# jscant/PointVS

Measured on AMD Instinct MI355X. Metric: protein-ligand graphs/sec fwd+bwd (+Adam step), 3-layer EGNN ch=32, ~2k nodes r=10A, higher is better.
Workload: dtype f32

## Files before the change

### pointvs_amd/csrc/graph_prepare.hip

```cpp
#include "common.h"
#include "profile.h"
#include <hipcub/hipcub.hpp>

namespace {

__global__ void k_extract(const int64_t* __restrict__ ei, const int64_t* __restrict__ ea, int A,
                          int N, int E, int32_t* row32, int32_t* col32, int32_t* ids,
                          uint8_t* etype_in, int32_t* status) {
    int e = blockIdx.x * blockDim.x + threadIdx.x;
    if (e >= E) return;
    int64_t r = ei[e], c = ei[(size_t)E + e];
    int bad = 0;
    if (r < 0 || r >= N || c < 0 || c >= N) { bad |= 1; r = 0; c = 0; }
    row32[e] = (int32_t)r;
    col32[e] = (int32_t)c;
    ids[e] = e;
    if (A > 0) {
        int hot = -1, ones = 0, other = 0;
        for (int a = 0; a < A; ++a) {
            int64_t v = ea[(size_t)e * A + a];
            if (v == 1) { ones++; hot = a; }
            else if (v != 0) other = 1;
        }
        if (ones != 1 || other) { bad |= 2; if (hot < 0) hot = 0; }
        etype_in[e] = (uint8_t)hot;
    }
    if (bad) atomicOr(status, bad);
}

__global__ void k_gather_sorted(const int32_t* __restrict__ perm, const int32_t* __restrict__ col32,
                                const uint8_t* __restrict__ etype_in, int E, int32_t* col,
                                uint8_t* etype, int32_t* iota) {
    int p = blockIdx.x * blockDim.x + threadIdx.x;
    if (p >= E) return;
    int e = perm[p];
    col[p] = col32[e];
    if (etype) etype[p] = etype_in[e];
    iota[p] = p;
}

__global__ void k_lower_bounds(const int32_t* __restrict__ keys, int E, int N, int32_t* ptr,
                               float* inv_deg) {
    int r = blockIdx.x * blockDim.x + threadIdx.x;
    if (r > N) return;
    auto lb = [&](int key) {
        int lo = 0, hi = E;
        while (lo < hi) {
            int mid = (lo + hi) >> 1;
            if (keys[mid] < key) lo = mid + 1; else hi = mid;
        }
        return lo;
    };
    int p0 = lb(r);
    ptr[r] = p0;
    if (inv_deg && r < N) {
        int deg = lb(r + 1) - p0;
        inv_deg[r] = 1.0f / (float)(deg > 1 ? deg : 1);
    }
}

int key_bits(int n) {
    int b = 1;
    while ((1ll << b) < (long long)n) ++b;
    return b;
}

size_t sort_temp_bytes(int E, int bits) {
    size_t bytes = 0;
    hipcub::DeviceRadixSort::SortPairs(nullptr, bytes, (const int32_t*)nullptr, (int32_t*)nullptr,
                                       (const int32_t*)nullptr, (int32_t*)nullptr, E, 0, bits, 0);
    return bytes;
}

struct PrepWs {
    int32_t *row32, *col32, *ids, *iota, *keys_tmp;
    uint8_t* etype_in;
    void* sort_tmp;
    size_t sort_bytes;
};

size_t carve(PvsArena& a, int N, int E, PrepWs* w) {
    size_t e = (size_t)(E > 0 ? E : 1);
    PrepWs t;
    t.row32 = a.take<int32_t>(e);
    t.col32 = a.take<int32_t>(e);
    t.ids = a.take<int32_t>(e);
    t.iota = a.take<int32_t>(e);
    t.keys_tmp = a.take<int32_t>(e);
    t.etype_in = a.take<uint8_t>(e);
    t.sort_bytes = sort_temp_bytes(E > 0 ? E : 1, key_bits(N > 1 ? N : 2));
    t.sort_tmp = a.take<char>(t.sort_bytes);
    if (w) *w = t;
    return a.off;
}

}

extern "C" size_t pvs_graph_prepare_workspace_bytes(int32_t n_nodes, int32_t n_edges) {
    PvsArena a(nullptr, 0);
    return carve(a, n_nodes, n_edges, nullptr) + 256;
}

extern "C" int pvs_graph_prepare(const int64_t* edge_index, const int64_t* edge_attr,
                                 int32_t n_edge_attr, int32_t N, int32_t E, int32_t* rowptr,
                                 int32_t* row, int32_t* col, uint8_t* etype, int32_t* perm,
                                 int32_t* colptr, int32_t* cedge, float* inv_deg, int32_t* status,
                                 void* workspace, size_t workspace_bytes, pvs_stream_t stream_) {
    hipStream_t stream = (hipStream_t)stream_;
    PVS_REQUIRE(N > 0 && E >= 0, "pvs_graph_prepare: bad sizes N=%d E=%d", N, E);
    PVS_REQUIRE(n_edge_attr >= 0 && n_edge_attr <= 255, "pvs_graph_prepare: bad n_edge_attr %d",
                n_edge_attr);
    PVS_REQUIRE(n_edge_attr == 0 || E == 0 || (edge_attr && etype), "pvs_graph_prepare: edge_attr/etype NULL");
    PVS_REQUIRE((colptr == nullptr) == (cedge == nullptr), "pvs_graph_prepare: colptr and cedge go together");
    PvsArena arena(workspace, workspace_bytes);
    PrepWs w;
    carve(arena, N, E, &w);
    PVS_REQUIRE(arena.ok(), "pvs_graph_prepare: workspace too small (%zu < %zu)", workspace_bytes,
                arena.off);
    PvsProfScope prof(stream, PVS_PROF_PREPARE);
    PVS_CHECK_HIP(hipMemsetAsync(status, 0, sizeof(int32_t), stream));
    const int bits = key_bits(N > 1 ? N : 2);
    const int T = 256;
    if (E > 0) {
        k_extract<<<(E + T - 1) / T, T, 0, stream>>>(edge_index, edge_attr, n_edge_attr, N, E,
                                                     w.row32, w.col32, w.ids, w.etype_in, status);
        PVS_CHECK_LAUNCH();
        size_t tb = w.sort_bytes;
        PVS_CHECK_HIP(hipcub::DeviceRadixSort::SortPairs(w.sort_tmp, tb, w.row32, row, w.ids, perm,
                                                         E, 0, bits, stream));
        k_gather_sorted<<<(E + T - 1) / T, T, 0, stream>>>(perm, w.col32, w.etype_in, E, col,
                                                           n_edge_attr ? etype : nullptr, w.iota);
        PVS_CHECK_LAUNCH();
        if (cedge) {
            tb = w.sort_bytes;
            PVS_CHECK_HIP(hipcub::DeviceRadixSort::SortPairs(w.sort_tmp, tb, col, w.keys_tmp, w.iota,
                                                             cedge, E, 0, bits, stream));
        }
    }
    k_lower_bounds<<<(N + 1 + T - 1) / T, T, 0, stream>>>(row, E, N, rowptr, inv_deg);
    PVS_CHECK_LAUNCH();
    if (cedge) {
        k_lower_bounds<<<(N + 1 + T - 1) / T, T, 0, stream>>>(w.keys_tmp, E, N, colptr, nullptr);
        PVS_CHECK_LAUNCH();
    }
    return 0;
}

namespace {

__device__ __forceinline__ int graph_of_edge(const int32_t* __restrict__ edge_ptr, int n_graphs, int e, int E,
                                             int edges_per_thread = 1) {
    __shared__ int g_first;
    if (threadIdx.x == 0) {
        const int e0 = min((int)(blockIdx.x * blockDim.x) * edges_per_thread, E - 1);
        int lo = 0, hi = n_graphs;
        while (hi - lo > 1) {
            const int mid = (lo + hi) >> 1;
            if (edge_ptr[mid] <= e0) lo = mid; else hi = mid;
        }
        g_first = lo;
    }
    __syncthreads();
    int g = g_first;
    while (g + 1 < n_graphs && edge_ptr[g + 1] <= e) ++g;
    return g;
}

template <bool VEC>
__global__ void k_extract_runs(const int64_t* __restrict__ ei, const int64_t* __restrict__ ea, int A, int N, int E,
                               int n_graphs, const int32_t* __restrict__ node_ptr, const int32_t* __restrict__ edge_ptr,
                               int32_t* __restrict__ row32, int32_t* __restrict__ col32, uint8_t* __restrict__ etype_in,
                               int32_t* __restrict__ split, int32_t* __restrict__ status) {
    const int e0 = 2 * (blockIdx.x * blockDim.x + threadIdx.x);
    int g = graph_of_edge(edge_ptr, n_graphs, min(e0, E - 1), E, 2);
    if (e0 >= E) return;
    const int n_here = e0 + 1 < E ? 2 : 1;
    int64_t rr[2], cc[2];
    if (VEC) {
        const longlong2 r2 = *reinterpret_cast<const longlong2*>(ei + e0);
        const longlong2 c2 = *reinterpret_cast<const longlong2*>(ei + (size_t)E + e0);
        rr[0] = r2.x; rr[1] = r2.y; cc[0] = c2.x; cc[1] = c2.y;
    } else {
        rr[0] = ei[e0]; cc[0] = ei[(size_t)E + e0];
        rr[1] = n_here > 1 ? ei[e0 + 1] : 0; cc[1] = n_here > 1 ? ei[(size_t)E + e0 + 1] : 0;
    }
    int64_t prev = e0 > 0 ? ei[e0 - 1] : 0;
    int hot[2] = {-1, -1}, attr_bad[2] = {0, 0};
    if (A > 0) {
        int ones[2] = {0, 0};
        if (VEC) {
            const longlong2* src = reinterpret_cast<const longlong2*>(ea + (size_t)e0 * A);
            for (int q = 0; q < A; ++q) {
                const longlong2 v = src[q];
                const int w0 = 2 * q, w1 = 2 * q + 1;
                const int ed0 = w0 >= A, ed1 = w1 >= A;
                if (v.x == 1) { ones[ed0]++; hot[ed0] = w0 - ed0 * A; } else if (v.x != 0) attr_bad[ed0] = 1;
                if (v.y == 1) { ones[ed1]++; hot[ed1] = w1 - ed1 * A; } else if (v.y != 0) attr_bad[ed1] = 1;
            }
        } else {
            for (int i = 0; i < n_here; ++i)
                for (int a = 0; a < A; ++a) {
                    const int64_t v = ea[(size_t)(e0 + i) * A + a];
                    if (v == 1) { ones[i]++; hot[i] = a; } else if (v != 0) attr_bad[i] = 1;
                }
        }
        for (int i = 0; i < 2; ++i) if (ones[i] != 1) attr_bad[i] = 1;
    }
    int bad = 0;
    int32_t r32[2] = {0, 0}, c32[2] = {0, 0};
    uint8_t ty[2] = {0, 0};
    for (int i = 0; i < n_here; ++i) {
        const int e = e0 + i;
        while (g + 1 < n_graphs && edge_ptr[g + 1] <= e) ++g;
        int64_t r = rr[i], c = cc[i];
        if (r < 0 || r >= N || c < 0 || c >= N) { bad |= 1; r = 0; c = 0; }
        if (r < node_ptr[g] || r >= node_ptr[g + 1] || c < node_ptr[g] || c >= node_ptr[g + 1]) bad |= 4;
        if (e < edge_ptr[g] || e >= edge_ptr[g + 1]) bad |= 4;
        if (e == 0 && (edge_ptr[0] != 0 || edge_ptr[n_graphs] != E || node_ptr[0] != 0 || node_ptr[n_graphs] != N)) bad |= 4;
        if (e > edge_ptr[g] && prev > rr[i]) {
            const int old = atomicMin(&split[g], e);
            if (old != edge_ptr[g + 1]) bad |= 4;
        }
        prev = rr[i];
        r32[i] = (int32_t)r; c32[i] = (int32_t)c;
        if (A > 0) {
            if (attr_bad[i]) { bad |= 2; if (hot[i] < 0) hot[i] = 0; }
            ty[i] = (uint8_t)hot[i];
        }
    }
    if (n_here == 2) {
        *reinterpret_cast<int2*>(row32 + e0) = make_int2(r32[0], r32[1]);
        *reinterpret_cast<int2*>(col32 + e0) = make_int2(c32[0], c32[1]);
        if (A > 0) *reinterpret_cast<uchar2*>(etype_in + e0) = make_uchar2(ty[0], ty[1]);
    } else {
        row32[e0] = r32[0]; col32[e0] = c32[0];
        if (A > 0) etype_in[e0] = ty[0];
    }
    if (bad) atomicOr(status, bad);
}

__global__ void k_iota(int E, int32_t* iota) {
    int p = blockIdx.x * blockDim.x + threadIdx.x;
    if (p < E) iota[p] = p;
}

__global__ void k_init_split(int n_graphs, const int32_t* __restrict__ edge_ptr, int32_t* __restrict__ split,
                             int32_t* __restrict__ status) {
    const int g = blockIdx.x * blockDim.x + threadIdx.x;
    if (g == 0) *status = 0;
    if (g < n_graphs) split[g] = edge_ptr[g + 1];
}

__global__ void k_run_starts(const int32_t* __restrict__ row32, int N, int E, int n_graphs,
                             const int32_t* __restrict__ status, const int32_t* __restrict__ node_ptr,
                             const int32_t* __restrict__ edge_ptr, const int32_t* __restrict__ split,
                             int32_t* __restrict__ start_a, int32_t* __restrict__ start_b, int32_t* __restrict__ cnt_a,
                             int32_t* __restrict__ rowptr, float* __restrict__ inv_deg) {
    const int n = blockIdx.x * blockDim.x + threadIdx.x;
    if (n >= N) return;
    if (n == N - 1) rowptr[N] = E;
    if (*status & 4) {
        start_a[n] = 0; start_b[n] = 0; cnt_a[n] = 0;
        rowptr[n] = n == 0 ? 0 : E;
        inv_deg[n] = 1.0f;
        return;
    }
    int lo = 0, hi = n_graphs;
    while (hi - lo > 1) {
        const int mid = (lo + hi) >> 1;
        if (node_ptr[mid] <= n) lo = mid; else hi = mid;
    }
    const int g = lo;
    const int a0 = edge_ptr[g], a1 = split[g], b1 = edge_ptr[g + 1];
    int f0 = a0, l0 = a1, f1 = a0, l1 = a1, f2 = a1, l2 = b1, f3 = a1, l3 = b1;
    while (f0 < l0 || f1 < l1 || f2 < l2 || f3 < l3) {
        const int m0 = (f0 + l0) >> 1, m1 = (f1 + l1) >> 1, m2 = (f2 + l2) >> 1, m3 = (f3 + l3) >> 1;
        const int v0 = f0 < l0 ? row32[m0] : 0, v1 = f1 < l1 ? row32[m1] : 0;
        const int v2 = f2 < l2 ? row32[m2] : 0, v3 = f3 < l3 ? row32[m3] : 0;
        if (f0 < l0) { if (v0 < n) f0 = m0 + 1; else l0 = m0; }
        if (f1 < l1) { if (v1 < n + 1) f1 = m1 + 1; else l1 = m1; }
        if (f2 < l2) { if (v2 < n) f2 = m2 + 1; else l2 = m2; }
        if (f3 < l3) { if (v3 < n + 1) f3 = m3 + 1; else l3 = m3; }
    }
    const int sa = f0, sa_next = f1, sb = f2, sb_next = f3;
    start_a[n] = sa;
    start_b[n] = sb;
    cnt_a[n] = sa_next - sa;
    const int d = (sa_next - sa) + (sb_next - sb);
    rowptr[n] = a0 + (sa - a0) + (sb - a1);
    inv_deg[n] = 1.0f / (float)(d > 1 ? d : 1);
}

__global__ void k_place_runs(const int32_t* __restrict__ row32, const int32_t* __restrict__ col32,
                             const uint8_t* __restrict__ etype_in, int E, int n_graphs,
                             const int32_t* __restrict__ edge_ptr, const int32_t* __restrict__ split,
                             const int32_t* __restrict__ rowptr, const int32_t* __restrict__ start_a,
                             const int32_t* __restrict__ start_b, const int32_t* __restrict__ cnt_a,
                             int32_t* __restrict__ row, int32_t* __restrict__ col, uint8_t* __restrict__ etype,
                             int32_t* __restrict__ perm, const int32_t* __restrict__ status) {
    const int e = blockIdx.x * blockDim.x + threadIdx.x;
    const int g = graph_of_edge(edge_ptr, n_graphs, min(e, E - 1), E);
    if (e >= E) return;
    if (*status & 4) {
        row[e] = 0; col[e] = 0; perm[e] = e;
        if (etype) etype[e] = 0;
        return;
    }
    const int r = row32[e];
    const bool second = e >= split[g];
    const int off = second ? e - start_b[r] : e - start_a[r];
    const int local = second ? cnt_a[r] + off : off;
    const int pos = rowptr[r] + local;
    row[pos] = r;
    col[pos] = col32[e];
    if (etype) etype[pos] = etype_in[e];
    perm[pos] = e;
}


constexpr int kCscMaxCols = 4096;
constexpr int kCscWaves = 4;
constexpr int kCscTargetChunks = 2048;
constexpr int kCscAhead = 8;

struct CscChunk { int begin, end, node_lo, width, g; };

__device__ __forceinline__ CscChunk csc_chunk(int wid, int cpg, int stride, int n_graphs, int N, int E,
                                              const int32_t* __restrict__ node_ptr,
                                              const int32_t* __restrict__ edge_ptr) {
    CscChunk c;
    c.g = wid / cpg;
    const int k = wid - c.g * cpg;
    if (c.g >= n_graphs) { c.begin = c.end = 0; c.node_lo = 0; c.width = 0; return c; }
    const int e0 = min(max(edge_ptr[c.g], 0), E), e1 = min(max(edge_ptr[c.g + 1], e0), E);
    const int len = (((e1 - e0) + cpg - 1) / cpg + 63) & ~63;
    c.begin = min(e0 + k * len, e1);
    c.end = min(c.begin + len, e1);
    c.node_lo = min(max(node_ptr[c.g], 0), N);
    c.width = min(max(node_ptr[c.g + 1], c.node_lo), N) - c.node_lo;
    return c;
}

template <class T, class Sink>
__device__ __forceinline__ void csc_walk_chunk(const int32_t* __restrict__ col, const CscChunk& c, int lane, T* tab,
                                               unsigned char* tag, Sink&& sink) {
    for (int q0 = c.begin; q0 < c.end; q0 += 64 * kCscAhead) {
        int keys[kCscAhead];
#pragma unroll
        for (int u = 0; u < kCscAhead; ++u)
            keys[u] = col[min(q0 + 64 * u + lane, c.end - 1)];
#pragma unroll
        for (int u = 0; u < kCscAhead; ++u) {
            const int k = min(max(keys[u] - c.node_lo, 0), c.width - 1);
            keys[u] = q0 + 64 * u + lane < c.end ? k : -1;
        }
#pragma unroll
        for (int u = 0; u < kCscAhead; ++u) {
            const int p = q0 + 64 * u + lane;
            const int key = keys[u];
            const bool live = key >= 0;
            if (q0 + 64 * u >= c.end) break;
            int leader = lane, rank = 0, members = 1;
            if (live) tag[key] = (unsigned char)lane;
            __builtin_amdgcn_fence(__ATOMIC_RELEASE, "wavefront");
            __builtin_amdgcn_wave_barrier();
            __builtin_amdgcn_fence(__ATOMIC_ACQUIRE, "wavefront");
            const bool lost = live && tag[key] != (unsigned char)lane;
            unsigned long long pending = __ballot(lost);
            while (pending) {
                const int l0 = __builtin_ctzll(pending);
                const int k0 = __builtin_amdgcn_readlane(key, l0);
                const unsigned long long grp = __ballot(live && key == k0);
                if (live && key == k0) {
                    leader = __builtin_ctzll(grp);
                    rank = __popcll(grp & ((1ull << lane) - 1ull));
                    members = __popcll(grp);
                }
                pending &= ~grp;
            }
            int slot = 0;
            if (live && rank == 0) {
                slot = (int)tab[key];
                tab[key] = (T)(slot + members);
            }
            slot = __shfl(slot, leader, 64) + rank;
            if (live) sink(slot, p);
            __builtin_amdgcn_fence(__ATOMIC_RELEASE, "wavefront");
            __builtin_amdgcn_wave_barrier();
            __builtin_amdgcn_fence(__ATOMIC_ACQUIRE, "wavefront");
        }
    }
}

template <bool PLACE>
__global__ void __launch_bounds__(64 * kCscWaves)
k_csc_pass(const int32_t* __restrict__ col, int n_graphs, int N, int E, const int32_t* __restrict__ node_ptr,
           const int32_t* __restrict__ edge_ptr, int cpg, int stride, int32_t* __restrict__ cnt,
           int32_t* __restrict__ cedge, int32_t* __restrict__ status) {
    extern __shared__ int32_t csc_lds[];
    const int lane = threadIdx.x & 63, wv = threadIdx.x >> 6;
    const int bpg = cpg / kCscWaves;
    const int xcd = blockIdx.x & 7, j = blockIdx.x >> 3;
    const int g_of_block = (j / bpg) * 8 + xcd;
    const int wid = g_of_block * cpg + (j % bpg) * kCscWaves + wv;
    CscChunk c = csc_chunk(g_of_block < n_graphs ? wid : n_graphs * cpg, cpg, stride, n_graphs, N, E, node_ptr, edge_ptr);
    if (c.width > stride) {
        if (lane == 0) atomicOr(status, 4);
        c.width = stride;
    }
    if (c.width <= 0) return;
    if (PLACE && (*status & 4)) {
        for (int p = c.begin + lane; p < c.end; p += 64) cedge[p] = p;
        return;
    }
    int32_t* tab = csc_lds + wv * (stride + stride / 4);
    unsigned char* tag = reinterpret_cast<unsigned char*>(tab + stride);
    int32_t* mine = cnt + (size_t)wid * stride;
    for (int i = lane; i < c.width; i += 64) tab[i] = PLACE ? mine[i] : 0;
    __builtin_amdgcn_fence(__ATOMIC_RELEASE, "wavefront");
    __builtin_amdgcn_wave_barrier();
    __builtin_amdgcn_fence(__ATOMIC_ACQUIRE, "wavefront");
    if (PLACE) {
        csc_walk_chunk(col, c, lane, tab, tag, [&](int slot, int p) { cedge[min(max(slot, 0), E - 1)] = p; });
        return;
    }
    for (int q0 = c.begin; q0 < c.end; q0 += 64 * kCscAhead) {
        int keys[kCscAhead];
#pragma unroll
        for (int u = 0; u < kCscAhead; ++u)
            keys[u] = col[min(q0 + 64 * u + lane, c.end - 1)];
#pragma unroll
        for (int u = 0; u < kCscAhead; ++u) {
            if (q0 + 64 * u >= c.end) break;
            const int k = min(max(keys[u] - c.node_lo, 0), c.width - 1);
            if (q0 + 64 * u + lane < c.end) atomicAdd(&tab[k], 1);
        }
    }
    if (!PLACE) {
        __builtin_amdgcn_fence(__ATOMIC_RELEASE, "wavefront");
        __builtin_amdgcn_wave_barrier();
        __builtin_amdgcn_fence(__ATOMIC_ACQUIRE, "wavefront");
        for (int i = lane; i < c.width; i += 64) mine[i] = tab[i];
    }
}

template <int NW>
__global__ void __launch_bounds__(64 * NW)
k_csc_place_tiles(const int32_t* __restrict__ col, int n_graphs, int N, int E, const int32_t* __restrict__ node_ptr,
                  const int32_t* __restrict__ edge_ptr, int cpg, int stride, const int32_t* __restrict__ cnt,
                  const int32_t* __restrict__ colptr, int32_t* __restrict__ cedge, int32_t* __restrict__ status, int cap) {
    extern __shared__ int32_t csc_lds[];
    const int lane = threadIdx.x & 63, wv = threadIdx.x >> 6, tid = threadIdx.x;
    const int tpg = cpg / NW;
    const int g = blockIdx.x / tpg, tl = blockIdx.x - g * tpg;
    if (g >= n_graphs) return;
    const int k0 = g * cpg + tl * NW;
    CscChunk c = csc_chunk(k0 + wv, cpg, stride, n_graphs, N, E, node_ptr, edge_ptr);
    if (c.width > stride) {
        if (lane == 0) atomicOr(status, 4);
        c.width = stride;
    }
    if (c.width <= 0) return;
    if (*status & 4) {
        for (int p = c.begin + lane; p < c.end; p += 64) cedge[p] = p;
        return;
    }
    const CscChunk first = csc_chunk(k0, cpg, stride, n_graphs, N, E, node_ptr, edge_ptr);
    const CscChunk last = csc_chunk(k0 + NW - 1, cpg, stride, n_graphs, N, E, node_ptr, edge_ptr);
    const int tile_begin = first.begin, tile_len = last.end - first.begin;
    const int width = c.width;
    if (tile_len > cap || tile_len > 65535) {
        int32_t* tab = csc_lds + wv * (stride + stride / 4);
        unsigned char* tag = reinterpret_cast<unsigned char*>(tab + stride);
        const int32_t* mine = cnt + (size_t)(k0 + wv) * stride;
        for (int i = lane; i < width; i += 64) tab[i] = mine[i];
        __builtin_amdgcn_fence(__ATOMIC_RELEASE, "wavefront");
        __builtin_amdgcn_wave_barrier();
        __builtin_amdgcn_fence(__ATOMIC_ACQUIRE, "wavefront");
        csc_walk_chunk(col, c, lane, tab, tag, [&](int slot, int p) { cedge[min(max(slot, 0), E - 1)] = p; });
        return;
    }
    int32_t* lstart = csc_lds;
    int32_t* gbase = lstart + stride + 64;
    unsigned short* tabs = reinterpret_cast<unsigned short*>(gbase + stride);
    unsigned char* tags = reinterpret_cast<unsigned char*>(tabs + NW * stride);
    unsigned short* list = reinterpret_cast<unsigned short*>(tags + NW * stride);
    const bool last_tile = tl == tpg - 1;
    for (int i = tid; i < width; i += 64 * NW) {
        const int32_t* src = cnt + (size_t)k0 * stride + i;
        const int s0 = src[0];
        const int s_end = last_tile ? colptr[c.node_lo + i + 1] : src[(size_t)NW * stride];
        gbase[i] = s0;
        lstart[i] = s_end - s0;
#pragma unroll
        for (int k = 0; k < NW; ++k) tabs[k * stride + i] = (unsigned short)(src[(size_t)k * stride] - s0);
    }
    __syncthreads();
    {
        __shared__ int32_t wave_tot[NW];
        const int per = (width + 64 * NW - 1) / (64 * NW), a = tid * per;
        int sum = 0;
        for (int i = a; i < min(a + per, width); ++i) sum += lstart[i];
        int inc = sum;
#pragma unroll
        for (int o = 1; o < 64; o <<= 1) {
            const int up = __shfl_up(inc, o, 64);
            if (lane >= o) inc += up;
        }
        if (lane == 63) wave_tot[wv] = inc;
        __syncthreads();
        int run = inc - sum;
        for (int k = 0; k < wv; ++k) run += wave_tot[k];
        for (int i = a; i < min(a + per, width); ++i) {
            const int v = lstart[i];
            lstart[i] = run;
            run += v;
        }
        if (tid == 64 * NW - 1) lstart[width] = run;
    }
    __syncthreads();
    for (int i = tid; i < width; i += 64 * NW) {
        const int base = lstart[i];
#pragma unroll
        for (int k = 0; k < NW; ++k) tabs[k * stride + i] = (unsigned short)(tabs[k * stride + i] + base);
    }
    __syncthreads();
    csc_walk_chunk(col, c, lane, tabs + wv * stride, tags + wv * stride,
                   [&](int slot, int p) { list[min(max(slot, 0), cap - 1)] = (unsigned short)(p - tile_begin); });
    __syncthreads();
    const int hw = tid >> 5, l32 = tid & 31;
    for (int cc = hw; cc < width; cc += 2 * NW) {
        const int a = lstart[cc], b = lstart[cc + 1], dst = gbase[cc];
        for (int i = a + l32; i < b; i += 32)
            cedge[min(max(dst + i - a, 0), E - 1)] = tile_begin + (int)list[min(i, cap - 1)];
    }
}

__device__ __forceinline__ int csc_graph_of_node(const int32_t* __restrict__ node_ptr, int n_graphs, int n) {
    int lo = 0, hi = n_graphs;
    while (hi - lo > 1) {
        const int mid = (lo + hi) >> 1;
        if (node_ptr[mid] <= n) lo = mid; else hi = mid;
    }
    return lo;
}

int csc_chunks_per_graph(int n_graphs) {
    int cpg = kCscTargetChunks / (n_graphs > 0 ? n_graphs : 1);
    cpg = (cpg / kCscWaves) * kCscWaves;
    if (cpg < kCscWaves) cpg = kCscWaves;
    if (cpg > 128) cpg = 128;
    return cpg;
}
int csc_blocks(int n_graphs, int cpg) { return ((n_graphs + 7) / 8) * (cpg / kCscWaves) * 8; }
int csc_stride(int max_graph_nodes) { return (max_graph_nodes + 63) & ~63; }
bool csc_counting_ok(int max_graph_nodes) { return max_graph_nodes > 0 && max_graph_nodes <= kCscMaxCols; }

struct RunsWs {
    int32_t *row32, *col32, *iota, *keys_tmp, *split, *start_a, *start_b, *cnt_a, *deg, *csc_cnt, *indeg;
    uint8_t* etype_in;
    void *sort_tmp, *scan_tmp;
    size_t sort_bytes, scan_bytes;
};

size_t carve_runs(PvsArena& a, int N, int E, int B, int max_graph_nodes, RunsWs* w) {
    const size_t e = (size_t)(E > 0 ? E : 1);
    RunsWs t;
    t.row32 = a.take<int32_t>(e);
    t.col32 = a.take<int32_t>(e);
    t.iota = a.take<int32_t>(e);
    t.keys_tmp = a.take<int32_t>(e);
    t.etype_in = a.take<uint8_t>(e);
    t.split = a.take<int32_t>((size_t)B + 1);
    t.start_a = a.take<int32_t>((size_t)N);
    t.start_b = a.take<int32_t>((size_t)N);
    t.cnt_a = a.take<int32_t>((size_t)N);
    t.deg = a.take<int32_t>((size_t)N + 1);
    t.sort_bytes = sort_temp_bytes(E > 0 ? E : 1, key_bits(N > 1 ? N : 2));
    t.sort_tmp = a.take<char>(t.sort_bytes);
    t.scan_bytes = 0;
    hipcub::DeviceScan::ExclusiveSum(nullptr, t.scan_bytes, (const int32_t*)nullptr, (int32_t*)nullptr, N + 1, 0);
    t.scan_tmp = a.take<char>(t.scan_bytes);
    t.csc_cnt = nullptr;
    t.indeg = nullptr;
    if (csc_counting_ok(max_graph_nodes)) {
        t.csc_cnt = a.take<int32_t>((size_t)B * csc_chunks_per_graph(B) * csc_stride(max_graph_nodes));
        t.indeg = a.take<int32_t>((size_t)N + 1);
    }
    if (w) *w = t;
    return a.off;
}

__global__ void k_csc_totals(const int32_t* __restrict__ cnt, int N, int n_graphs, const int32_t* __restrict__ node_ptr,
                             int cpg, int stride, int32_t* __restrict__ indeg, const int32_t* __restrict__ status) {
    const int n = blockIdx.x * blockDim.x + threadIdx.x;
    if (n >= N) return;
    if (*status & 4) { indeg[n] = 0; return; }
    const int g = csc_graph_of_node(node_ptr, n_graphs, n);
    const int c = n - node_ptr[g];
    int t0 = 0, t1 = 0, t2 = 0, t3 = 0;
    if (c >= 0 && c < stride) {
        const int32_t* src = cnt + (size_t)g * cpg * stride + c;
        for (int k = 0; k < cpg; k += 4) {
            t0 += src[(size_t)k * stride];
            t1 += src[(size_t)(k + 1) * stride];
            t2 += src[(size_t)(k + 2) * stride];
            t3 += src[(size_t)(k + 3) * stride];
        }
    }
    indeg[n] = (t0 + t1) + (t2 + t3);
}

__global__ void __launch_bounds__(256) k_csc_colptr(int32_t* __restrict__ cnt, const int32_t* __restrict__ indeg, int N, int E,
                                                    int n_graphs, const int32_t* __restrict__ node_ptr,
                                                    const int32_t* __restrict__ edge_ptr, int cpg, int stride,
                                                    int32_t* __restrict__ colptr, const int32_t* __restrict__ status) {
    __shared__ int32_t wave_tot[4], front_tot[4];
    const int t = threadIdx.x, lane = t & 63, wv = t >> 6;
    if (*status & 4) {
        for (int i = (blockIdx.y * gridDim.x + blockIdx.x) * 256 + t; i <= N; i += gridDim.x * gridDim.y * 256) colptr[i] = 0;
        return;
    }
    for (int g = blockIdx.y; g < n_graphs; g += gridDim.y) {
        if (g == n_graphs - 1 && blockIdx.x == 0 && t == 0) colptr[N] = E;
        const int n0 = node_ptr[g], width = min(node_ptr[g + 1] - n0, stride);
        const int c0 = blockIdx.x * 256;
        if (c0 >= width) continue;
        int front = 0;
        for (int c = t; c < c0; c += 256) front += indeg[n0 + c];
        const int c = c0 + t;
        const int mine = c < width ? indeg[n0 + c] : 0;
        int inc = mine;
#pragma unroll
        for (int o = 1; o < 64; o <<= 1) {
            const int up = __shfl_up(inc, o, 64);
            if (lane >= o) inc += up;
            front += __shfl_xor(front, o, 64);
        }
        if (lane == 63) wave_tot[wv] = inc;
        if (lane == 0) front_tot[wv] = front;
        __syncthreads();
        int run = edge_ptr[g] + (front_tot[0] + front_tot[1]) + (front_tot[2] + front_tot[3]) + inc - mine;
        for (int k = 0; k < wv; ++k) run += wave_tot[k];
        if (c < width) {
            colptr[n0 + c] = run;
            int32_t* slot = cnt + (size_t)g * cpg * stride + c;
            for (int k = 0; k < cpg; k += 4) {
                const int v0 = slot[(size_t)k * stride], v1 = slot[(size_t)(k + 1) * stride];
                const int v2 = slot[(size_t)(k + 2) * stride], v3 = slot[(size_t)(k + 3) * stride];
                slot[(size_t)k * stride] = run;
                slot[(size_t)(k + 1) * stride] = run + v0;
                slot[(size_t)(k + 2) * stride] = run + v0 + v1;
                slot[(size_t)(k + 3) * stride] = run + v0 + v1 + v2;
                run += (v0 + v1) + (v2 + v3);
            }
        }
        __syncthreads();
    }
}

}

extern "C" size_t pvs_graph_prepare_runs_workspace_bytes(int32_t n_nodes, int32_t n_edges, int32_t n_graphs,
                                                         int32_t max_graph_nodes) {
    PvsArena a(nullptr, 0);
    return carve_runs(a, n_nodes, n_edges, n_graphs, max_graph_nodes, nullptr) + 256;
}

extern "C" int pvs_graph_prepare_runs(const int64_t* edge_index, const int64_t* edge_attr, int32_t n_edge_attr,
                                      int32_t N, int32_t E, int32_t n_graphs, const int32_t* node_ptr,
                                      const int32_t* edge_ptr, int32_t* rowptr, int32_t* row, int32_t* col,
                                      uint8_t* etype, int32_t* perm, int32_t* colptr, int32_t* cedge, float* inv_deg,
                                      int32_t* status, int32_t max_graph_nodes, void* workspace,
                                      size_t workspace_bytes, pvs_stream_t stream_) {
    hipStream_t stream = (hipStream_t)stream_;
    PVS_REQUIRE(N > 0 && E >= 0 && n_graphs > 0, "pvs_graph_prepare_runs: bad sizes N=%d E=%d B=%d", N, E, n_graphs);
    PVS_REQUIRE(max_graph_nodes >= 0, "pvs_graph_prepare_runs: bad max_graph_nodes %d", max_graph_nodes);
    PVS_REQUIRE(n_edge_attr >= 0 && n_edge_attr <= 255, "pvs_graph_prepare_runs: bad n_edge_attr %d", n_edge_attr);
    PVS_REQUIRE(n_edge_attr == 0 || (edge_attr && etype), "pvs_graph_prepare_runs: edge_attr/etype NULL");
    PVS_REQUIRE(node_ptr && edge_ptr, "pvs_graph_prepare_runs: node_ptr / edge_ptr NULL");
    PVS_REQUIRE((colptr == nullptr) == (cedge == nullptr), "pvs_graph_prepare_runs: colptr and cedge go together");
    PvsArena arena(workspace, workspace_bytes);
    RunsWs w;
    carve_runs(arena, N, E, n_graphs, max_graph_nodes, &w);
    PVS_REQUIRE(arena.ok(), "pvs_graph_prepare_runs: workspace too small (%zu < %zu)", workspace_bytes, arena.off);
    PvsProfScope prof(stream, PVS_PROF_PREPARE);
    const int T = 256;
    k_init_split<<<(n_graphs + T - 1) / T > 0 ? (n_graphs + T - 1) / T : 1, T, 0, stream>>>(n_graphs, edge_ptr, w.split, status);
    PVS_CHECK_LAUNCH();
    if (E > 0) {
        const bool vec = (E & 1) == 0 && (((uintptr_t)edge_index | (uintptr_t)edge_attr) & 15) == 0;
        const int pairs = (E + 1) / 2;
        if (vec)
            k_extract_runs<true><<<(pairs + T - 1) / T, T, 0, stream>>>(edge_index, edge_attr, n_edge_attr, N, E, n_graphs,
                                                                        node_ptr, edge_ptr, w.row32, w.col32, w.etype_in,
                                                                        w.split, status);
        else
            k_extract_runs<false><<<(pairs + T - 1) / T, T, 0, stream>>>(edge_index, edge_attr, n_edge_attr, N, E, n_graphs,
                                                                         node_ptr, edge_ptr, w.row32, w.col32, w.etype_in,
                                                                         w.split, status);
        PVS_CHECK_LAUNCH();
    }
    k_run_starts<<<(N + T - 1) / T, T, 0, stream>>>(w.row32, N, E, n_graphs, status, node_ptr, edge_ptr, w.split, w.start_a,
                                                    w.start_b, w.cnt_a, rowptr, inv_deg);
    PVS_CHECK_LAUNCH();
    if (E > 0) {
        k_place_runs<<<(E + T - 1) / T, T, 0, stream>>>(w.row32, w.col32, w.etype_in, E, n_graphs, edge_ptr, w.split,
                                                        rowptr, w.start_a, w.start_b, w.cnt_a, row, col,
                                                        n_edge_attr ? etype : nullptr, perm, status);
        PVS_CHECK_LAUNCH();
    }
    if (!cedge) return 0;
    static const bool force_sort = [] { const char* e = getenv("PVS_CSC_SORT"); return e && e[0] == '1'; }();
    if (w.csc_cnt && !force_sort) {
        const int cpg = csc_chunks_per_graph(n_graphs), stride = csc_stride(max_graph_nodes);
        const int waves = n_graphs * cpg, blocks = csc_blocks(n_graphs, cpg);
        const size_t lds = (size_t)kCscWaves * (stride + stride / 4) * sizeof(int32_t);
        if (lds > 48 * 1024) {
            PVS_CHECK_HIP(hipFuncSetAttribute((const void*)k_csc_pass<false>, hipFuncAttributeMaxDynamicSharedMemorySize, (int)lds));
            PVS_CHECK_HIP(hipFuncSetAttribute((const void*)k_csc_pass<true>, hipFuncAttributeMaxDynamicSharedMemorySize, (int)lds));
        }
        if (E > 0) {
            k_csc_pass<false><<<blocks, 64 * kCscWaves, lds, stream>>>(col, n_graphs, N, E, node_ptr, edge_ptr, cpg, stride,
                                                                        w.csc_cnt, nullptr, status);
            PVS_CHECK_LAUNCH();
        } else {
            PVS_CHECK_HIP(hipMemsetAsync(w.csc_cnt, 0, (size_t)waves * stride * sizeof(int32_t), stream));
        }
        k_csc_totals<<<(N + T - 1) / T, T, 0, stream>>>(w.csc_cnt, N, n_graphs, node_ptr, cpg, stride, w.indeg, status);
        PVS_CHECK_LAUNCH();
        k_csc_colptr<<<dim3((max_graph_nodes + 255) / 256, n_graphs < 65535 ? n_graphs : 65535), 256, 0, stream>>>(w.csc_cnt, w.indeg, N, E, n_graphs, node_ptr,
                                                                                         edge_ptr, cpg, stride, colptr, status);
        PVS_CHECK_LAUNCH();
        if (E > 0) {
            const char* tiles_env = getenv("PVS_CSC_TILES");
            const bool tiles_on = !(tiles_env && tiles_env[0] == '0');
            const int budget = 160 * 1024 - 256;
            auto fixed_bytes = [&](int nw) { return (size_t)(stride + 64) * 4 + (size_t)stride * 4 + (size_t)nw * stride * 3; };
            int nw = (cpg % 8 == 0 && fixed_bytes(8) + 2 * 32768 <= (size_t)budget) ? 8 : 4;
            int cap = ((int)budget - (int)fixed_bytes(nw)) / 2;
            if (cap > 65535) cap = 65535;
            const bool forced = tiles_env && tiles_env[0] == '2';
            const double avg_run = (double)E / ((double)(N > 0 ? N : 1) * (double)(cpg / nw));
            if (tiles_on && (avg_run >= 10.0 || forced) && cap >= 8192 && (size_t)nw * (stride + stride / 4) * 4 <= (size_t)budget) {
                const int tiles = n_graphs * (cpg / nw);
                if (nw == 8) {
                    PVS_CHECK_HIP(hipFuncSetAttribute((const void*)k_csc_place_tiles<8>, hipFuncAttributeMaxDynamicSharedMemorySize, budget));
                    k_csc_place_tiles<8><<<tiles, 64 * 8, budget, stream>>>(col, n_graphs, N, E, node_ptr, edge_ptr, cpg, stride,
                                                                           w.csc_cnt, colptr, cedge, status, cap);
                } else {
                    PVS_CHECK_HIP(hipFuncSetAttribute((const void*)k_csc_place_tiles<4>, hipFuncAttributeMaxDynamicSharedMemorySize, budget));
                    k_csc_place_tiles<4><<<tiles, 64 * 4, budget, stream>>>(col, n_graphs, N, E, node_ptr, edge_ptr, cpg, stride,
                                                                           w.csc_cnt, colptr, cedge, status, cap);
                }
            } else {
                k_csc_pass<true><<<blocks, 64 * kCscWaves, lds, stream>>>(col, n_graphs, N, E, node_ptr, edge_ptr, cpg, stride,
                                                                           w.csc_cnt, cedge, status);
            }
            PVS_CHECK_LAUNCH();
        }
        return 0;
    }
    if (E > 0) {
        size_t tb = w.sort_bytes;
        const int bits = key_bits(N > 1 ? N : 2);
        k_iota<<<(E + 255) / 256, 256, 0, stream>>>(E, w.iota);
        PVS_CHECK_LAUNCH();
        PVS_CHECK_HIP(hipcub::DeviceRadixSort::SortPairs(w.sort_tmp, tb, col, w.keys_tmp, w.iota, cedge, E, 0,
                                                         bits, stream));
    }
    k_lower_bounds<<<(N + 1 + T - 1) / T, T, 0, stream>>>(w.keys_tmp, E, N, colptr, nullptr);
    PVS_CHECK_LAUNCH();
    return 0;
}

namespace {
}

size_t pvs_build_csc_workspace_bytes(int N, int E) {
    const size_t e = (size_t)(E > 0 ? E : 1);
    return 2 * pvs_align_up(e * sizeof(int32_t), 256) +
           pvs_align_up(sort_temp_bytes((int)e, key_bits(N > 1 ? N : 2)), 256) + 512;
}

int pvs_build_csc(hipStream_t stream, const int32_t* col, int E, int N, int32_t* colptr, int32_t* cedge,
                  void* workspace, size_t workspace_bytes) {
    PVS_REQUIRE(workspace_bytes >= pvs_build_csc_workspace_bytes(N, E) - 512, "build_csc: workspace too small");
    PvsArena a(workspace, workspace_bytes);
    const size_t e = (size_t)(E > 0 ? E : 1);
    int32_t* iota = a.take<int32_t>(e);
    int32_t* keys = a.take<int32_t>(e);
    const int bits = key_bits(N > 1 ? N : 2);
    size_t tb = sort_temp_bytes((int)e, bits);
    void* tmp = a.take<char>(tb);
    if (E > 0) {
        k_iota<<<(E + 255) / 256, 256, 0, stream>>>(E, iota);
        PVS_CHECK_LAUNCH();
        PVS_CHECK_HIP(hipcub::DeviceRadixSort::SortPairs(tmp, tb, col, keys, iota, cedge, E, 0, bits, stream));
    }
    k_lower_bounds<<<(N + 1 + 255) / 256, 256, 0, stream>>>(keys, E, N, colptr, nullptr);
    PVS_CHECK_LAUNCH();
    return 0;
}

namespace {
template <bool FILL>
__global__ void __launch_bounds__(256)
k_filter_ligand(PvsGraph g, const uint8_t* __restrict__ bp, int capacity, int32_t* __restrict__ cnt,
                const int32_t* __restrict__ rowptr_out, int32_t* __restrict__ row_out,
                int32_t* __restrict__ col_out, uint8_t* __restrict__ etype_out, int32_t* __restrict__ status) {
    const int lane = threadIdx.x & 63;
    const int i = (blockIdx.x * 256 + threadIdx.x) >> 6;
    if (i >= g.n_nodes) return;
    const bool lig_row = bp[i] == 0;
    const int p0 = g.rowptr[i], p1 = g.rowptr[i + 1];
    int done = 0;
    const int base = FILL ? rowptr_out[i] : 0;
    if (FILL && rowptr_out[g.n_nodes] > capacity) {
        if (i == 0 && lane == 0) atomicOr(status, 4);
        return;
    }
    for (int pb = p0; pb < p1; pb += 64) {
        const int p = pb + lane;
        int c = 0;
        bool keep = false;
        if (p < p1) {
            c = g.col[p];
            keep = lig_row || bp[c] == 0;
        }
        const unsigned long long m = __ballot(keep);
        if (FILL && keep) {
            const int q = base + done + __popcll(m & ((1ull << lane) - 1ull));
            row_out[q] = i;
            col_out[q] = c;
            if (etype_out) etype_out[q] = g.etype[p];
        }
        done += __popcll(m);
    }
    if (!FILL && lane == 0) cnt[i] = done;
}
}

extern "C" size_t pvs_graph_filter_workspace_bytes(int32_t N) {
    size_t sb = 0;
    (void)hipcub::DeviceScan::ExclusiveSum(nullptr, sb, (const int32_t*)nullptr, (int32_t*)nullptr, N + 1);
    return pvs_align_up(((size_t)N + 1) * sizeof(int32_t), 256) + pvs_align_up(sb, 256) + 512;
}

extern "C" int pvs_graph_filter_ligand_edges(const PvsGraph* full, const uint8_t* bp, int32_t capacity,
                                             int32_t* rowptr_out, int32_t* row_out, int32_t* col_out,
                                             uint8_t* etype_out, int32_t* status, void* workspace,
                                             size_t workspace_bytes, pvs_stream_t stream_) {
    hipStream_t s = (hipStream_t)stream_;
    PVS_REQUIRE(full && bp && rowptr_out && row_out && col_out && status && full->rowptr && full->col,
                "pvs_graph_filter_ligand_edges: NULL");
    PVS_REQUIRE(!full->n_edges_dev, "pvs_graph_filter_ligand_edges: needs a graph with a host-side edge count");
    PVS_REQUIRE(etype_out == nullptr || full->etype, "pvs_graph_filter_ligand_edges: graph has no edge classes");
    const int N = full->n_nodes;
    PVS_REQUIRE(workspace_bytes >= pvs_graph_filter_workspace_bytes(N) - 512, "filter workspace too small");
    PvsArena a(workspace, workspace_bytes);
    int32_t* cnt = a.take<int32_t>((size_t)N + 1);
    size_t sb = 0;
// ... 145 lines not shown
```

Before: 5809.

## Drop staging arrays in edge prep: scan rows, then place directly from int64 input

The extract pass that wrote row32/col32/etype staging arrays is replaced by a light row-only scan that finds each graph's split point. The placement kernel now reads int64 edge_index and edge_attr directly, with nontemporal loads and a wave-level LDS transpose of attr codes, and uses a per-node int2 offset record instead of three per-node arrays. This removes one full write-then-read of edge data and several workspace buffers, but edge attributes are validated later. Status bit 1 now also forces the fallback layout, and bad columns are replaced with the row index.

New measurement: 5882, median of 6. 1.01x the previous value.

```diff
diff --git a/pointvs_amd/csrc/graph_prepare.hip b/pointvs_amd/csrc/graph_prepare.hip
--- a/pointvs_amd/csrc/graph_prepare.hip
+++ b/pointvs_amd/csrc/graph_prepare.hip
@@ -166,75 +166,66 @@
     return g;
 }
 
-template <bool VEC>
-__global__ void k_extract_runs(const int64_t* __restrict__ ei, const int64_t* __restrict__ ea, int A, int N, int E,
-                               int n_graphs, const int32_t* __restrict__ node_ptr, const int32_t* __restrict__ edge_ptr,
-                               int32_t* __restrict__ row32, int32_t* __restrict__ col32, uint8_t* __restrict__ etype_in,
-                               int32_t* __restrict__ split, int32_t* __restrict__ status) {
-    const int e0 = 2 * (blockIdx.x * blockDim.x + threadIdx.x);
-    int g = graph_of_edge(edge_ptr, n_graphs, min(e0, E - 1), E, 2);
-    if (e0 >= E) return;
-    const int n_here = e0 + 1 < E ? 2 : 1;
-    int64_t rr[2], cc[2];
-    if (VEC) {
-        const longlong2 r2 = *reinterpret_cast<const longlong2*>(ei + e0);
-        const longlong2 c2 = *reinterpret_cast<const longlong2*>(ei + (size_t)E + e0);
-        rr[0] = r2.x; rr[1] = r2.y; cc[0] = c2.x; cc[1] = c2.y;
-    } else {
-        rr[0] = ei[e0]; cc[0] = ei[(size_t)E + e0];
-        rr[1] = n_here > 1 ? ei[e0 + 1] : 0; cc[1] = n_here > 1 ? ei[(size_t)E + e0 + 1] : 0;
-    }
-    int64_t prev = e0 > 0 ? ei[e0 - 1] : 0;
-    int hot[2] = {-1, -1}, attr_bad[2] = {0, 0};
-    if (A > 0) {
-        int ones[2] = {0, 0};
-        if (VEC) {
-            const longlong2* src = reinterpret_cast<const longlong2*>(ea + (size_t)e0 * A);
-            for (int q = 0; q < A; ++q) {
-                const longlong2 v = src[q];
-                const int w0 = 2 * q, w1 = 2 * q + 1;
-                const int ed0 = w0 >= A, ed1 = w1 >= A;
-                if (v.x == 1) { ones[ed0]++; hot[ed0] = w0 - ed0 * A; } else if (v.x != 0) attr_bad[ed0] = 1;
-                if (v.y == 1) { ones[ed1]++; hot[ed1] = w1 - ed1 * A; } else if (v.y != 0) attr_bad[ed1] = 1;
-            }
-        } else {
-            for (int i = 0; i < n_here; ++i)
-                for (int a = 0; a < A; ++a) {
-                    const int64_t v = ea[(size_t)(e0 + i) * A + a];
-                    if (v == 1) { ones[i]++; hot[i] = a; } else if (v != 0) attr_bad[i] = 1;
-                }
-        }
-        for (int i = 0; i < 2; ++i) if (ones[i] != 1) attr_bad[i] = 1;
-    }
+constexpr int kScanEdges = 8;
+constexpr int kPlaceEdges = 4;
+constexpr int kPrepThreads = 256;
+constexpr int kPrepWaves = kPrepThreads / 64;
+
+typedef long long pvs_ll2 __attribute__((ext_vector_type(2)));
+template <class T> __device__ __forceinline__ T prep_load_once(const T* p) { return __builtin_nontemporal_load(p); }
+
+struct PrepSeg { int g, n_lo, n_hi, e_lo, e_hi; };
+
+__device__ __forceinline__ void prep_seg_load(PrepSeg& s, const int32_t* __restrict__ node_ptr,
+                                              const int32_t* __restrict__ edge_ptr) {
+    s.n_lo = node_ptr[s.g]; s.n_hi = node_ptr[s.g + 1];
+    s.e_lo = edge_ptr[s.g]; s.e_hi = edge_ptr[s.g + 1];
+}
+
+__device__ __forceinline__ bool prep_seg_advance(PrepSeg& s, int e, int n_graphs, const int32_t* __restrict__ node_ptr,
+                                                 const int32_t* __restrict__ edge_ptr) {
+    if (s.g + 1 >= n_graphs || s.e_hi > e) return false;
+    do ++s.g; while (s.g + 1 < n_graphs && edge_ptr[s.g + 1] <= e);
+    prep_seg_load(s, node_ptr, edge_ptr);
+    return true;
+}
+
+__global__ void __launch_bounds__(kPrepThreads)
+k_scan_rows(const int64_t* __restrict__ rows, int N, int E, int n_graphs, const int32_t* __restrict__ node_ptr,
+            const int32_t* __restrict__ edge_ptr, int32_t* __restrict__ split, int32_t* __restrict__ status) {
+    const int lane = threadIdx.x & 63, wv = threadIdx.x >> 6;
+    const long long cb = ((long long)blockIdx.x * kPrepWaves + wv) * (64 * kScanEdges);
+    PrepSeg s;
+    s.g = graph_of_edge(edge_ptr, n_graphs, (int)min(cb + lane, (long long)E - 1), E, kScanEdges);
+    if (cb >= E) return;
+    long long r[kScanEdges];
+#pragma unroll
+    for (int j = 0; j < kScanEdges; ++j) {
+        const long long e = cb + 64 * j + lane;
+        r[j] = e < E ? (long long)rows[e] : 0;
+    }
+    long long before = 0;
+    if (lane == 0 && cb > 0) before = rows[cb - 1];
+    prep_seg_load(s, node_ptr, edge_ptr);
     int bad = 0;
-    int32_t r32[2] = {0, 0}, c32[2] = {0, 0};
-    uint8_t ty[2] = {0, 0};
-    for (int i = 0; i < n_here; ++i) {
-        const int e = e0 + i;
-        while (g + 1 < n_graphs && edge_ptr[g + 1] <= e) ++g;
-        int64_t r = rr[i], c = cc[i];
-        if (r < 0 || r >= N || c < 0 || c >= N) { bad |= 1; r = 0; c = 0; }
-        if (r < node_ptr[g] || r >= node_ptr[g + 1] || c < node_ptr[g] || c >= node_ptr[g + 1]) bad |= 4;
-        if (e < edge_ptr[g] || e >= edge_ptr[g + 1]) bad |= 4;
+#pragma unroll
+    for (int j = 0; j < kScanEdges; ++j) {
+        long long prev = __shfl_up(r[j], 1, 64);
+        const long long carry = j ? __shfl(r[j ? j - 1 : 0], 63, 64) : before;
+        if (lane == 0) prev = carry;
+        const long long el = cb + 64 * j + lane;
+        if (el >= E) continue;
+        const int e = (int)el;
+        prep_seg_advance(s, e, n_graphs, node_ptr, edge_ptr);
+        long long v = r[j];
+        if (v < 0 || v >= N) { bad |= 1; v = 0; }
+        if (v < s.n_lo || v >= s.n_hi) bad |= 4;
+        if (e < s.e_lo || e >= s.e_hi) bad |= 4;
         if (e == 0 && (edge_ptr[0] != 0 || edge_ptr[n_graphs] != E || node_ptr[0] != 0 || node_ptr[n_graphs] != N)) bad |= 4;
-        if (e > edge_ptr[g] && prev > rr[i]) {
-            const int old = atomicMin(&split[g], e);
-            if (old != edge_ptr[g + 1]) bad |= 4;
-        }
-        prev = rr[i];
-        r32[i] = (int32_t)r; c32[i] = (int32_t)c;
-        if (A > 0) {
-            if (attr_bad[i]) { bad |= 2; if (hot[i] < 0) hot[i] = 0; }
-            ty[i] = (uint8_t)hot[i];
-        }
-    }
-    if (n_here == 2) {
-        *reinterpret_cast<int2*>(row32 + e0) = make_int2(r32[0], r32[1]);
-        *reinterpret_cast<int2*>(col32 + e0) = make_int2(c32[0], c32[1]);
-        if (A > 0) *reinterpret_cast<uchar2*>(etype_in + e0) = make_uchar2(ty[0], ty[1]);
-    } else {
-        row32[e0] = r32[0]; col32[e0] = c32[0];
-        if (A > 0) etype_in[e0] = ty[0];
+        if (e > s.e_lo && prev > r[j]) {
+            const int old = atomicMin(&split[s.g], e);
+            if (old != s.e_hi) bad |= 4;
+        }
     }
     if (bad) atomicOr(status, bad);
 }
@@ -251,16 +242,18 @@
     if (g < n_graphs) split[g] = edge_ptr[g + 1];
 }
 
-__global__ void k_run_starts(const int32_t* __restrict__ row32, int N, int E, int n_graphs,
+__global__ void k_run_starts(const int64_t* __restrict__ rows, int N, int E, int n_graphs,
                              const int32_t* __restrict__ status, const int32_t* __restrict__ node_ptr,
                              const int32_t* __restrict__ edge_ptr, const int32_t* __restrict__ split,
-                             int32_t* __restrict__ start_a, int32_t* __restrict__ start_b, int32_t* __restrict__ cnt_a,
+                             int2* __restrict__ rec, int32_t* __restrict__ unsafe,
                              int32_t* __restrict__ rowptr, float* __restrict__ inv_deg) {
     const int n = blockIdx.x * blockDim.x + threadIdx.x;
     if (n >= N) return;
     if (n == N - 1) rowptr[N] = E;
-    if (*status & 4) {
-        start_a[n] = 0; start_b[n] = 0; cnt_a[n] = 0;
+    const bool broken = (*status & 5) != 0;
+    if (n == 0) *unsafe = broken;
+    if (broken) {
+        rec[n] = make_int2(0, 0);
         rowptr[n] = n == 0 ? 0 : E;
         inv_deg[n] = 1.0f;
         return;
@@ -275,48 +268,117 @@
     int f0 = a0, l0 = a1, f1 = a0, l1 = a1, f2 = a1, l2 = b1, f3 = a1, l3 = b1;
     while (f0 < l0 || f1 < l1 || f2 < l2 || f3 < l3) {
         const int m0 = (f0 + l0) >> 1, m1 = (f1 + l1) >> 1, m2 = (f2 + l2) >> 1, m3 = (f3 + l3) >> 1;
-        const int v0 = f0 < l0 ? row32[m0] : 0, v1 = f1 < l1 ? row32[m1] : 0;
-        const int v2 = f2 < l2 ? row32[m2] : 0, v3 = f3 < l3 ? row32[m3] : 0;
+        const int64_t v0 = f0 < l0 ? rows[m0] : 0, v1 = f1 < l1 ? rows[m1] : 0;
+        const int64_t v2 = f2 < l2 ? rows[m2] : 0, v3 = f3 < l3 ? rows[m3] : 0;
         if (f0 < l0) { if (v0 < n) f0 = m0 + 1; else l0 = m0; }
         if (f1 < l1) { if (v1 < n + 1) f1 = m1 + 1; else l1 = m1; }
         if (f2 < l2) { if (v2 < n) f2 = m2 + 1; else l2 = m2; }
         if (f3 < l3) { if (v3 < n + 1) f3 = m3 + 1; else l3 = m3; }
     }
     const int sa = f0, sa_next = f1, sb = f2, sb_next = f3;
-    start_a[n] = sa;
-    start_b[n] = sb;
-    cnt_a[n] = sa_next - sa;
     const int d = (sa_next - sa) + (sb_next - sb);
-    rowptr[n] = a0 + (sa - a0) + (sb - a1);
+    const int first = a0 + (sa - a0) + (sb - a1);
+    rowptr[n] = first;
+    rec[n] = make_int2(first - sa, first + (sa_next - sa) - sb);
     inv_deg[n] = 1.0f / (float)(d > 1 ? d : 1);
 }
 
-__global__ void k_place_runs(const int32_t* __restrict__ row32, const int32_t* __restrict__ col32,
-                             const uint8_t* __restrict__ etype_in, int E, int n_graphs,
-                             const int32_t* __restrict__ edge_ptr, const int32_t* __restrict__ split,
-                             const int32_t* __restrict__ rowptr, const int32_t* __restrict__ start_a,
-                             const int32_t* __restrict__ start_b, const int32_t* __restrict__ cnt_a,
-                             int32_t* __restrict__ row, int32_t* __restrict__ col, uint8_t* __restrict__ etype,
-                             int32_t* __restrict__ perm, const int32_t* __restrict__ status) {
-    const int e = blockIdx.x * blockDim.x + threadIdx.x;
-    const int g = graph_of_edge(edge_ptr, n_graphs, min(e, E - 1), E);
-    if (e >= E) return;
-    if (*status & 4) {
-        row[e] = 0; col[e] = 0; perm[e] = e;
-        if (etype) etype[e] = 0;
-        return;
-    }
-    const int r = row32[e];
-    const bool second = e >= split[g];
-    const int off = second ? e - start_b[r] : e - start_a[r];
-    const int local = second ? cnt_a[r] + off : off;
-    const int pos = rowptr[r] + local;
-    row[pos] = r;
-    col[pos] = col32[e];
-    if (etype) etype[pos] = etype_in[e];
-    perm[pos] = e;
-}
-
+__device__ __forceinline__ int prep_code(long long v) { return v == 0 ? 0 : v == 1 ? 1 : 2; }
+
+template <bool VEC, int AMAX>
+__global__ void __launch_bounds__(kPrepThreads)
+k_place_stream(const int64_t* __restrict__ ei, const int64_t* __restrict__ ea, int A, int N, int E, int n_graphs,
+               const int32_t* __restrict__ node_ptr, const int32_t* __restrict__ edge_ptr,
+               const int32_t* __restrict__ split, const int2* __restrict__ rec, const int32_t* __restrict__ unsafe,
+               int32_t* __restrict__ row, int32_t* __restrict__ col, uint8_t* __restrict__ etype,
+               int32_t* __restrict__ perm, int32_t* __restrict__ status) {
+    __shared__ unsigned short codes[kPrepWaves][kPlaceEdges / 2][64 * AMAX];
+    const int lane = threadIdx.x & 63, wv = threadIdx.x >> 6;
+    const long long cb = ((long long)blockIdx.x * kPrepWaves + wv) * (64 * kPlaceEdges);
+    PrepSeg s;
+    s.g = graph_of_edge(edge_ptr, n_graphs, (int)min(cb + lane, (long long)E - 1), E, kPlaceEdges);
+    if (cb >= E) return;
+    const int64_t* cols = ei + (size_t)E;
+    long long r[kPlaceEdges], c[kPlaceEdges];
+#pragma unroll
+    for (int j = 0; j < kPlaceEdges; ++j) {
+        const long long e = cb + 64 * j + lane;
+        r[j] = e < E ? (long long)prep_load_once(ei + e) : 0;
+        c[j] = e < E ? (long long)prep_load_once(cols + e) : 0;
+    }
+    const bool by_pieces = A > 0 && A <= AMAX;
+    if (by_pieces) {
+        const size_t words = (size_t)E * A;
+        pvs_ll2 av[kPlaceEdges / 2][AMAX];
+#pragma unroll
+        for (int jj = 0; jj < kPlaceEdges / 2; ++jj)
+#pragma unroll
+            for (int q = 0; q < AMAX; ++q) {
+                av[jj][q] = pvs_ll2{0, 0};
+                if (q >= A) continue;
+                const size_t w0 = (size_t)(cb + 128 * jj) * A + 2 * (size_t)(q * 64 + lane);
+                if (VEC && w0 + 1 < words) {
+                    av[jj][q] = prep_load_once(reinterpret_cast<const pvs_ll2*>(ea + w0));
+                } else {
+                    if (w0 < words) av[jj][q].x = ea[w0];
+                    if (w0 + 1 < words) av[jj][q].y = ea[w0 + 1];
+                }
+            }
+#pragma unroll
+        for (int jj = 0; jj < kPlaceEdges / 2; ++jj)
+#pragma unroll
+            for (int q = 0; q < AMAX; ++q)
+                if (q < A) codes[wv][jj][q * 64 + lane] = (unsigned short)(prep_code(av[jj][q].x) | prep_code(av[jj][q].y) << 8);
+        __builtin_amdgcn_fence(__ATOMIC_RELEASE, "wavefront");
+        __builtin_amdgcn_wave_barrier();
+        __builtin_amdgcn_fence(__ATOMIC_ACQUIRE, "wavefront");
+    }
+    const bool safe_graph = *unsafe != 0;
+    prep_seg_load(s, node_ptr, edge_ptr);
+    int second_from = split[s.g];
+    int bad = 0;
+#pragma unroll
+    for (int j = 0; j < kPlaceEdges; ++j) {
+        const long long el = cb + 64 * j + lane;
+        if (el >= E) continue;
+        const int e = (int)el;
+        if (prep_seg_advance(s, e, n_graphs, node_ptr, edge_ptr)) second_from = split[s.g];
+        long long cc = c[j];
+        bool col_bad = false;
+        if (cc < 0 || cc >= N) { bad |= 1; cc = 0; col_bad = true; }
+        if (cc < s.n_lo || cc >= s.n_hi) { bad |= 4; col_bad = true; }
+        int hot = -1;
+        if (A > 0) {
+            int ones = 0, other = 0;
+            if (by_pieces) {
+                const unsigned char* mine = reinterpret_cast<const unsigned char*>(codes[wv][j >> 1]) + ((j & 1) * 64 + lane) * A;
+                for (int a = 0; a < A; ++a) {
+                    const int k = mine[a];
+                    if (k == 1) { ones++; hot = a; } else if (k != 0) other = 1;
+                }
+            } else {
+                for (int a = 0; a < A; ++a) {
+                    const int64_t v = ea[(size_t)e * A + a];
+                    if (v == 1) { ones++; hot = a; } else if (v != 0) other = 1;
+                }
+            }
+            if (ones != 1 || other) { bad |= 2; if (hot < 0) hot = 0; }
+        }
+        if (safe_graph) {
+            row[e] = 0; col[e] = 0; perm[e] = e;
+            if (etype) etype[e] = 0;
+            continue;
+        }
+        const int rr = (int)r[j];
+        const int2 t = rec[rr];
+        const int pos = e + (e >= second_from ? t.y : t.x);
+        row[pos] = rr;
+        col[pos] = col_bad ? rr : (int)cc;
+        if (etype) etype[pos] = (uint8_t)hot;
+        perm[pos] = e;
+    }
+    if (bad) atomicOr(status, bad);
+}
 
 constexpr int kCscMaxCols = 4096;
 constexpr int kCscWaves = 4;
@@ -557,36 +619,31 @@
 bool csc_counting_ok(int max_graph_nodes) { return max_graph_nodes > 0 && max_graph_nodes <= kCscMaxCols; }
 
 struct RunsWs {
-    int32_t *row32, *col32, *iota, *keys_tmp, *split, *start_a, *start_b, *cnt_a, *deg, *csc_cnt, *indeg;
-    uint8_t* etype_in;
-    void *sort_tmp, *scan_tmp;
-    size_t sort_bytes, scan_bytes;
+    int32_t *iota, *keys_tmp, *split, *unsafe, *csc_cnt, *indeg;
+    int2* rec;
+    void* sort_tmp;
+    size_t sort_bytes;
 };
 
 size_t carve_runs(PvsArena& a, int N, int E, int B, int max_graph_nodes, RunsWs* w) {
     const size_t e = (size_t)(E > 0 ? E : 1);
     RunsWs t;
-    t.row32 = a.take<int32_t>(e);
-    t.col32 = a.take<int32_t>(e);
-    t.iota = a.take<int32_t>(e);
-    t.keys_tmp = a.take<int32_t>(e);
-    t.etype_in = a.take<uint8_t>(e);
     t.split = a.take<int32_t>((size_t)B + 1);
-    t.start_a = a.take<int32_t>((size_t)N);
-    t.start_b = a.take<int32_t>((size_t)N);
-    t.cnt_a = a.take<int32_t>((size_t)N);
-    t.deg = a.take<int32_t>((size_t)N + 1);
-    t.sort_bytes = sort_temp_bytes(E > 0 ? E : 1, key_bits(N > 1 ? N : 2));
-    t.sort_tmp = a.take<char>(t.sort_bytes);
-    t.scan_bytes = 0;
-    hipcub::DeviceScan::ExclusiveSum(nullptr, t.scan_bytes, (const int32_t*)nullptr, (int32_t*)nullptr, N + 1, 0);
-    t.scan_tmp = a.take<char>(t.scan_bytes);
+    t.unsafe = a.take<int32_t>(1);
+    t.rec = a.take<int2>((size_t)N);
     t.csc_cnt = nullptr;
     t.indeg = nullptr;
+    t.iota = t.keys_tmp = nullptr;
+    t.sort_tmp = nullptr;
+    t.sort_bytes = 0;
     if (csc_counting_ok(max_graph_nodes)) {
         t.csc_cnt = a.take<int32_t>((size_t)B * csc_chunks_per_graph(B) * csc_stride(max_graph_nodes));
         t.indeg = a.take<int32_t>((size_t)N + 1);
     }
+    t.iota = a.take<int32_t>(e);
+    t.keys_tmp = a.take<int32_t>(e);
+    t.sort_bytes = sort_temp_bytes(E > 0 ? E : 1, key_bits(N > 1 ? N : 2));
+    t.sort_tmp = a.take<char>(t.sort_bytes);
     if (w) *w = t;
     return a.off;
 }
@@ -689,25 +746,23 @@
     k_init_split<<<(n_graphs + T - 1) / T > 0 ? (n_graphs + T - 1) / T : 1, T, 0, stream>>>(n_graphs, edge_ptr, w.split, status);
     PVS_CHECK_LAUNCH();
     if (E > 0) {
-        const bool vec = (E & 1) == 0 && (((uintptr_t)edge_index | (uintptr_t)edge_attr) & 15) == 0;
-        const int pairs = (E + 1) / 2;
-        if (vec)
-            k_extract_runs<true><<<(pairs + T - 1) / T, T, 0, stream>>>(edge_index, edge_attr, n_edge_attr, N, E, n_graphs,
-                                                                        node_ptr, edge_ptr, w.row32, w.col32, w.etype_in,
-                                                                        w.split, status);
-        else
-            k_extract_runs<false><<<(pairs + T - 1) / T, T, 0, stream>>>(edge_index, edge_attr, n_edge_attr, N, E, n_graphs,
-                                                                         node_ptr, edge_ptr, w.row32, w.col32, w.etype_in,
-                                                                         w.split, status);
+        const int scan_edges = kPrepThreads * kScanEdges;
+        k_scan_rows<<<(E + scan_edges - 1) / scan_edges, kPrepThreads, 0, stream>>>(edge_index, N, E, n_graphs, node_ptr,
+                                                                                           edge_ptr, w.split, status);
         PVS_CHECK_LAUNCH();
     }
-    k_run_starts<<<(N + T - 1) / T, T, 0, stream>>>(w.row32, N, E, n_graphs, status, node_ptr, edge_ptr, w.split, w.start_a,
-                                                    w.start_b, w.cnt_a, rowptr, inv_deg);
+    k_run_starts<<<(N + T - 1) / T, T, 0, stream>>>(edge_index, N, E, n_graphs, status, node_ptr, edge_ptr, w.split, w.rec,
+                                                    w.unsafe, rowptr, inv_deg);
     PVS_CHECK_LAUNCH();
     if (E > 0) {
-        k_place_runs<<<(E + T - 1) / T, T, 0, stream>>>(w.row32, w.col32, w.etype_in, E, n_graphs, edge_ptr, w.split,
-                                                        rowptr, w.start_a, w.start_b, w.cnt_a, row, col,
-                                                        n_edge_attr ? etype : nullptr, perm, status);
+        const bool vec = ((uintptr_t)edge_attr & 15) == 0;
+        const int place_edges = kPrepThreads * kPlaceEdges;
+        const int blocks = (E + place_edges - 1) / place_edges;
+        auto place = n_edge_attr <= 3 ? (vec ? k_place_stream<true, 3> : k_place_stream<false, 3>)
+                                      : (vec ? k_place_stream<true, 8> : k_place_stream<false, 8>);
+        place<<<blocks, kPrepThreads, 0, stream>>>(edge_index, edge_attr, n_edge_attr, N, E, n_graphs, node_ptr, edge_ptr,
+                                                   w.split, w.rec, w.unsafe, row, col, n_edge_attr ? etype : nullptr, perm,
+                                                   status);
         PVS_CHECK_LAUNCH();
     }
     if (!cedge) return 0;
```
